# facebookresearch/metamorph

Hardware: AMD Instinct MI355X
Metric: train tokens/sec (LLaMA-3-8B + SigLIP-SO400M, seq2048, 256 img toks), whole job (higher is better)
Workload: dtype bf16

## Files before the change

metamorph_amd/csrc/gemm_bf16.hip:

```cpp
#include "gemm_common.h"
#include <type_traits>
#include <cstdlib>

namespace {

template <int TM, int TN, int FM, int FN>
MM_DEV void gemm_epilogue(f32x4 (&acc)[FM][FN], const GemmArgs& a, unsigned char* smem, int m0, int n0, int wm, int wn, int wave, int lane) {
    const int fr = lane & 15, fq = lane >> 4;
    const int M = a.M, N = a.N;
    constexpr int CPL = TN / 4;
    float* stg = (float*)smem + wave * (16 * TN);
    const uint32_t fl = a.flags;
    const int row_l = lane >> 2, col_l = (lane & 3) * CPL;
    uint16_t* Cb = (uint16_t*)a.C;
    float* Cf = (float*)a.C;
    const bool vec_ok = ((a.ldc & 7) == 0) && (!(fl & MM355_GEMM_RESIDUAL) || (a.ldr & 7) == 0);
#pragma unroll
    for (int i = 0; i < FM; ++i) {
        __builtin_amdgcn_fence(__ATOMIC_RELEASE, "wavefront");
        __builtin_amdgcn_wave_barrier();
#pragma unroll
        for (int j = 0; j < FN; ++j)
#pragma unroll
            for (int r = 0; r < 4; ++r) stg[(fq * 4 + r) * TN + j * 16 + fr] = acc[i][j][r];
// ... 8 lines not shown
                if (c >= N) continue;
                float v[8];
                const f32x4 s0 = *(const f32x4*)(stg + row_l * TN + col_l + j * 8);
                const f32x4 s1 = *(const f32x4*)(stg + row_l * TN + col_l + j * 8 + 4);
                v[0] = s0.x; v[1] = s0.y; v[2] = s0.z; v[3] = s0.w;
                v[4] = s1.x; v[5] = s1.y; v[6] = s1.z; v[7] = s1.w;
                epi_store8(a, fl, vec_ok, grow, rr, c, v);
            }
        }
    }
}

MM_DEV void gemm_epilogue_swiglu(f32x4 (&acc)[8][4], const GemmArgs& a, unsigned char* smem, int m0, int tn, int wm, int wn, int wave, int lane) {
    constexpr int TN = 64;
    const int fr = lane & 15, fq = lane >> 4;
    const int M = a.M, I = (int)a.res_mod;
    float* stg = (float*)smem + wave * (16 * TN);
    const int row_l = lane >> 2, k4 = lane & 3;
    uint16_t* gu = (uint16_t*)a.C;
    uint16_t* act = (uint16_t*)a.res;
    const int ch0 = tn * 128 + wn * 32;
#pragma unroll
    for (int i = 0; i < 8; ++i) {
        __builtin_amdgcn_fence(__ATOMIC_RELEASE, "wavefront");
        __builtin_amdgcn_wave_barrier();
#pragma unroll
        for (int j = 0; j < 4; ++j)
#pragma unroll
            for (int r = 0; r < 4; ++r) stg[(fq * 4 + r) * TN + j * 16 + fr] = acc[i][j][r];
        __builtin_amdgcn_fence(__ATOMIC_RELEASE, "wavefront");
        __builtin_amdgcn_wave_barrier();
        const int grow = m0 + wm * 128 + i * 16 + row_l;
        if (grow < M) {
            float g[8], u[8], o[8];
            const f32x4 g0 = *(const f32x4*)(stg + row_l * TN + k4 * 8), g1 = *(const f32x4*)(stg + row_l * TN + k4 * 8 + 4);
            const f32x4 u0 = *(const f32x4*)(stg + row_l * TN + 32 + k4 * 8), u1 = *(const f32x4*)(stg + row_l * TN + 32 + k4 * 8 + 4);
            g[0] = g0.x; g[1] = g0.y; g[2] = g0.z; g[3] = g0.w; g[4] = g1.x; g[5] = g1.y; g[6] = g1.z; g[7] = g1.w;
            u[0] = u0.x; u[1] = u0.y; u[2] = u0.z; u[3] = u0.w; u[4] = u1.x; u[5] = u1.y; u[6] = u1.z; u[7] = u1.w;
            const u32x4 gp = pack8(g), up = pack8(u);
            const int ch = ch0 + k4 * 8;
            *(u32x4*)(gu + (int64_t)grow * a.ldc + ch) = gp;
            *(u32x4*)(gu + (int64_t)grow * a.ldc + I + ch) = up;
            float gb[8], ub[8];
            unpack8(gp, gb);
            unpack8(up, ub);
#pragma unroll
            for (int e = 0; e < 8; ++e) o[e] = round_bf(gb[e] / (1.0f + __expf(-gb[e]))) * ub[e];
            *(u32x4*)(act + (int64_t)grow * a.ldr + ch) = pack8(o);
        }
    }
}

constexpr int SWB_TROW = 144;
constexpr int SWB_T = 3 * 32 * SWB_TROW;
constexpr int SWB_LDS = 32768 + 8 * SWB_T;
MM_DEV void gemm_epilogue_swiglu_bwd(f32x4 (&acc)[8][4], const GemmArgs& a, unsigned char* smem, int m0, int n0, int wm, int wn, int wave, int lane) {
    constexpr int TN = 64, PF = 4;
    typedef __attribute__((ext_vector_type(4))) short s16x4;
    typedef __attribute__((address_space(3))) s16x4* lds4_t;
    const int fr = lane & 15, fq = lane >> 4;
    const int M = a.M, I = a.N;
    float* stg = (float*)smem + wave * (16 * TN);
    unsigned char* tile = smem + 32768 + wave * SWB_T;
    const int row_l = lane >> 2, k4 = lane & 3;
    const uint16_t* gu = a.res;
    uint16_t* dgu = (uint16_t*)a.C;
    const int c_wave = n0 + wn * 64;
    if (c_wave >= I) return;
    const int row0 = m0 + wm * 128 + row_l;
    u32x4 gq[PF][2], uq[PF][2];
    auto fetch = [&](int i, int slot) {
        const int grow = row0 + i * 16;
#pragma unroll
        for (int j8 = 0; j8 < 2; ++j8) {
            const int64_t ro = (int64_t)min(grow, M - 1) * a.ldr + c_wave + k4 * 16 + j8 * 8;
            gq[slot][j8] = *(const u32x4*)(gu + ro);
            uq[slot][j8] = *(const u32x4*)(gu + ro + I);
        }
    };
#pragma unroll
    for (int i = 0; i < PF; ++i) fetch(i, i);
#pragma unroll
    for (int ib = 0; ib < 4; ++ib) {
#pragma unroll
        for (int half = 0; half < 2; ++half) {
            const int i = ib * 2 + half;
            __builtin_amdgcn_fence(__ATOMIC_RELEASE, "wavefront");
            __builtin_amdgcn_wave_barrier();
#pragma unroll
            for (int j = 0; j < 4; ++j)
#pragma unroll
                for (int r = 0; r < 4; ++r) stg[(fq * 4 + r) * TN + j * 16 + fr] = acc[i][j][r];
            __builtin_amdgcn_fence(__ATOMIC_RELEASE, "wavefront");
            __builtin_amdgcn_wave_barrier();
            const int grow = row0 + i * 16;
            const bool live = grow < M;
#pragma unroll
            for (int j8 = 0; j8 < 2; ++j8) {
                const int c = k4 * 16 + j8 * 8;
                float daf[8], g[8], u[8], dg[8], du[8], av[8], da[8];
                const f32x4 s0 = *(const f32x4*)(stg + row_l * TN + c), s1 = *(const f32x4*)(stg + row_l * TN + c + 4);
                daf[0] = s0.x; daf[1] = s0.y; daf[2] = s0.z; daf[3] = s0.w; daf[4] = s1.x; daf[5] = s1.y; daf[6] = s1.z; daf[7] = s1.w;
                unpack8(pack8(daf), da);
                unpack8(gq[i % PF][j8], g);
                unpack8(uq[i % PF][j8], u);
#pragma unroll
                for (int e = 0; e < 8; ++e) {
                    const float sg = 1.0f / (1.0f + __expf(-g[e]));
                    const float silu = g[e] * sg;
                    av[e] = round_bf(silu) * u[e];
                    du[e] = da[e] * round_bf(silu);
                    dg[e] = da[e] * u[e] * (sg * (1.0f + g[e] * (1.0f - sg)));
                }
                const u32x4 pg = pack8(dg), pu = pack8(du), pa = pack8(av);
                if (live) {
                    const int64_t wo = (int64_t)grow * a.ldc + c_wave + c;
                    *(u32x4*)(dgu + wo) = pg;
                    *(u32x4*)(dgu + wo + I) = pu;
                }
                unsigned char* tp = tile + (half * 16 + row_l) * SWB_TROW + c * 2;
                *(u32x4*)(tp) = pa;
                *(u32x4*)(tp + 32 * SWB_TROW) = pg;
                *(u32x4*)(tp + 64 * SWB_TROW) = pu;
            }
            if (i + PF < 8) fetch(i + PF, i % PF);
        }
        __builtin_amdgcn_fence(__ATOMIC_RELEASE, "wavefront");
        __builtin_amdgcn_wave_barrier();
        const int r_base = m0 + wm * 128 + ib * 32;
        const int s_l = fr >> 2, j_l = fr & 3;
        const unsigned char* tb = tile + (8 * (fr & 3) + (fr >> 2)) * SWB_TROW + fq * 8;
#pragma unroll
        for (int q = 0; q < 3; ++q) {
#pragma unroll
            for (int it = 0; it < 4; ++it) {
                const s16x4 lo = __builtin_amdgcn_ds_read_tr16_b64_v4i16((lds4_t)(tb + q * 32 * SWB_TROW + it * 32));
                const s16x4 hi = __builtin_amdgcn_ds_read_tr16_b64_v4i16((lds4_t)(tb + (q * 32 + 4) * SWB_TROW + it * 32));
                const int ch = c_wave + it * 16 + fq * 4 + j_l;
                const int r8 = r_base + 8 * s_l;
                if (r8 < M) {
                    typedef __attribute__((ext_vector_type(8))) short s16x8;
                    uint16_t* outp = (q == 0 ? a.aux0 : a.aux1) + (int64_t)(q == 2 ? I + ch : ch) * a.ld_aux;
                    *(s16x8*)(outp + r8) = s16x8{lo[0], lo[1], lo[2], lo[3], hi[0], hi[1], hi[2], hi[3]};
                }
            }
        }
    }
}

MM_DEV void gemm_epilogue_rope(f32x4 (&acc)[8][4], const GemmArgs& a, unsigned char* smem, int m0, int n0, int wm, int wn, int wave, int lane) {
    constexpr int TN = 64;
    const int fr = lane & 15, fq = lane >> 4;
    const int M = a.M, L = (int)a.ld_aux, n_rot = (int)a.res_mod;
    float* stg = (float*)smem + wave * (16 * TN);
    const int row_l = lane >> 2, k4 = lane & 3;
    uint16_t* out = (uint16_t*)a.C;
    const int32_t* pos_off = (const int32_t*)a.bias;
    const int d1 = (wn & 1) * 32 + k4 * 8;
    const int col1 = n0 + (wn >> 1) * 128 + d1;
    const bool rot = col1 < n_rot;
#pragma unroll
    for (int i = 0; i < 8; ++i) {
        __builtin_amdgcn_fence(__ATOMIC_RELEASE, "wavefront");
        __builtin_amdgcn_wave_barrier();
#pragma unroll
        for (int j = 0; j < 4; ++j)
#pragma unroll
            for (int r = 0; r < 4; ++r) stg[(fq * 4 + r) * TN + j * 16 + fr] = acc[i][j][r];
        __builtin_amdgcn_fence(__ATOMIC_RELEASE, "wavefront");
        __builtin_amdgcn_wave_barrier();
        const int grow = m0 + wm * 128 + i * 16 + row_l;
        if (grow < M) {
            float a1[8], a2[8], x1[8], x2[8];
            const f32x4 p0 = *(const f32x4*)(stg + row_l * TN + k4 * 8), p1 = *(const f32x4*)(stg + row_l * TN + k4 * 8 + 4);
            const f32x4 q0 = *(const f32x4*)(stg + row_l * TN + 32 + k4 * 8), q1 = *(const f32x4*)(stg + row_l * TN + 32 + k4 * 8 + 4);
            a1[0] = p0.x; a1[1] = p0.y; a1[2] = p0.z; a1[3] = p0.w; a1[4] = p1.x; a1[5] = p1.y; a1[6] = p1.z; a1[7] = p1.w;
            a2[0] = q0.x; a2[1] = q0.y; a2[2] = q0.z; a2[3] = q0.w; a2[4] = q1.x; a2[5] = q1.y; a2[6] = q1.z; a2[7] = q1.w;
            u32x4 w1 = pack8(a1), w2 = pack8(a2);
            if (rot) {
                unpack8(w1, x1);
                unpack8(w2, x2);
                const int b = grow / L;
                const int l = grow - b * L + (pos_off ? pos_off[b] : 0);
                float c[8], sn[8], y1[8], y2[8];
                unpack8(*(const u32x4*)(a.aux0 + (int64_t)l * 128 + d1), c);
                unpack8(*(const u32x4*)(a.aux1 + (int64_t)l * 128 + d1), sn);
#pragma unroll
                for (int e = 0; e < 8; ++e) {
                    y1[e] = round_bf(x1[e] * c[e]) + round_bf(-x2[e] * sn[e]);
                    y2[e] = round_bf(x2[e] * c[e]) + round_bf(x1[e] * sn[e]);
                }
                w1 = pack8(y1); w2 = pack8(y2);
            }
            *(u32x4*)(out + (int64_t)grow * a.ldc + col1) = w1;
            *(u32x4*)(out + (int64_t)grow * a.ldc + col1 + 64) = w2;
        }
    }
}

// ... 911 lines not shown

#ifdef MM355_LEGACY_VARIANTS
int launch_gemm_pp2(GemmArgs a, hipStream_t s) {
    if (!pp_eligible(a, false, false)) return launch_gemm<256, 256, 2, 4, true, 1, false>(a, s);
    static std::atomic<uint64_t> lds_ok{0};
    if (mm_ensure_dynamic_lds((const void*)gemm_pp2_kernel, PP_LDS, lds_ok) != MM355_OK) return MM355_ELAUNCH;
    const int64_t total = pp_prepare(a);
    if (total <= 0 || total > 0x7fffffff) return MM355_EINVAL;
    hipLaunchKernelGGL(gemm_pp2_kernel, dim3((unsigned)total), dim3(512), PP_LDS, s, a);
    return mm_launch_status();
}

#endif

int launch_gemm_pp(GemmArgs a, hipStream_t s) {
    if (!pp_eligible(a, false, false)) return launch_gemm<256, 256, 2, 4, true, 1, false>(a, s);
    return launch_gemm_pp_t<false, false>(a, s);
}

#ifdef MM355_LEGACY_VARIANTS
int launch_gemm_ring(GemmArgs a, hipStream_t s) {
    if (a.K < 128) return launch_gemm<256, 256, 2, 4, true, 0, false>(a, s);
    constexpr int LDS = 4 * (256 + 256) * 64;
    static std::atomic<uint64_t> lds_ok{0};
    if (mm_ensure_dynamic_lds((const void*)gemm_nt_ring_kernel, LDS, lds_ok) != MM355_OK) return MM355_ELAUNCH;
    a.ntm = (a.M + 255) / 256;
    a.ntn = (a.N + 255) / 256;
    const int64_t total = (int64_t)a.ntm * a.ntn;
    if (total <= 0 || total > 0x7fffffff) return MM355_EINVAL;
    hipLaunchKernelGGL(gemm_nt_ring_kernel, dim3((unsigned)total), dim3(512), LDS, s, a);
    return mm_launch_status();
}

#endif

template <int BM, int BN, int WM, int WN, bool GLDS, int PIPE = 0, bool TNL = false>
int launch_gemm(GemmArgs a, hipStream_t s) {
    constexpr int STAGE = (BM + BN) * 128;
    constexpr int LDS = 2 * STAGE;
    auto kern = gemm_nt_kernel<BM, BN, WM, WN, GLDS, PIPE, TNL>;
    static std::atomic<uint64_t> lds_ok{0};
    if (mm_ensure_dynamic_lds((const void*)kern, LDS, lds_ok) != MM355_OK) return MM355_ELAUNCH;
    a.ntm = (a.M + BM - 1) / BM;
    a.ntn = (a.N + BN - 1) / BN;
    const int64_t total = (int64_t)a.ntm * a.ntn;
    if (total <= 0 || total > 0x7fffffff) return MM355_EINVAL;
    hipLaunchKernelGGL(kern, dim3((unsigned)total), dim3(WM * WN * 64), LDS, s, a);
    return mm_launch_status();
}

__global__ __launch_bounds__(256) void transpose_kernel(const uint16_t* __restrict__ in, int64_t ld_in, int rows, int cols,
                                                        uint16_t* __restrict__ out, int64_t ld_out) {
    __shared__ uint16_t tile[64][64 + 2];
    const int r0 = blockIdx.y * 64, c0 = blockIdx.x * 64;
    const int tid = threadIdx.x;
#pragma unroll
    for (int i = 0; i < 2; ++i) {
        const int v = tid + i * 256, r = v >> 3, c = (v & 7) * 8;
        const int gr = r0 + r, gc = c0 + c;
        uint16_t tmp[8];
        if (gr < rows && gc + 8 <= cols) {
            *(u32x4*)tmp = *(const u32x4*)(in + (int64_t)gr * ld_in + gc);
        } else {
#pragma unroll
            for (int e = 0; e < 8; ++e) tmp[e] = (gr < rows && gc + e < cols) ? in[(int64_t)gr * ld_in + gc + e] : (uint16_t)0;
        }
#pragma unroll
        for (int e = 0; e < 8; ++e) tile[r][c + e] = tmp[e];
    }
    __syncthreads();
#pragma unroll
    for (int i = 0; i < 2; ++i) {
        const int v = tid + i * 256, c = v >> 3, r = (v & 7) * 8;
        const int gc = c0 + c, gr = r0 + r;
        if (gc >= cols) continue;
        uint16_t tmp[8];
#pragma unroll
        for (int e = 0; e < 8; ++e) tmp[e] = tile[r + e][c];
        if (gr + 8 <= rows && ((ld_out & 7) == 0)) {
            *(u32x4*)(out + (int64_t)gc * ld_out + gr) = *(const u32x4*)tmp;
        } else {
            for (int e = 0; e < 8; ++e)
                if (gr + e < rows) out[(int64_t)gc * ld_out + gr + e] = tmp[e];
        }
    }
}

__global__ __launch_bounds__(256) void colsum_kernel(const uint16_t* __restrict__ x, int64_t ld, int M, int N, float* __restrict__ out) {
    __shared__ float part[4][64];
    const int cq = threadIdx.x & 63, rp = threadIdx.x >> 6;
    const int c = blockIdx.x * 64 + cq;
    float s = 0.f;
    if (c < N)
        for (int r = rp; r < M; r += 4) s += bf2f(x[(int64_t)r * ld + c]);
    part[rp][cq] = s;
    __syncthreads();
    if (rp == 0 && c < N) out[c] += (part[0][cq] + part[1][cq]) + (part[2][cq] + part[3][cq]);
}

__global__ __launch_bounds__(1024) void colsum8_kernel(const uint16_t* __restrict__ x, int64_t ld, int M, int N, float* __restrict__ out) {
    __shared__ float part[128][65];
    const int cg = threadIdx.x & 7, rp = threadIdx.x >> 3;
    const int c0 = blockIdx.x * 64 + cg * 8;
    float s[8] = {0.f, 0.f, 0.f, 0.f, 0.f, 0.f, 0.f, 0.f};
    if (c0 < N)
        for (int r = rp; r < M; r += 128) {
            float f[8];
// ... 379 lines not shown
}
}

extern "C" int mm355_gemm_pair_bf16(const mm355_bf16* A0, int64_t lda0, const mm355_bf16* B0, int64_t ldb0, void* C0, int64_t ldc0,
                                    int64_t M0, int64_t N0, int64_t K0, uint32_t flags0,
                                    const mm355_bf16* A1, int64_t lda1, const mm355_bf16* B1, int64_t ldb1, void* C1, int64_t ldc1,
                                    int64_t M1, int64_t N1, int64_t K1, uint32_t flags1, void* stream) {
    (void)hipGetLastError();
    GemmArgs a0, a1;
    int rc = pair_problem(a0, A0, lda0, B0, ldb0, C0, ldc0, M0, N0, K0, flags0);
    if (rc != MM355_OK) return rc;
    rc = pair_problem(a1, A1, lda1, B1, ldb1, C1, ldc1, M1, N1, K1, flags1);
    if (rc != MM355_OK) return rc;
    return launch_gemm_pp_pair(a0, a1, (hipStream_t)stream);
}

extern "C" int mm355_gemm_tn_bf16(const mm355_bf16* At, int64_t lda, const mm355_bf16* Bt, int64_t ldb, void* C, int64_t ldc, int64_t M,
                                  int64_t N, int64_t K, uint32_t flags, void* stream) {
    (void)hipGetLastError();
    if (!At || !Bt || !C || M < 8 || N < 8 || K <= 0) return MM355_EINVAL;
    if ((M & 7) || (N & 7) || (lda & 7) || (ldb & 7) || !mm_aligned16(At) || !mm_aligned16(Bt) || !mm_aligned16(C)) return MM355_EINVAL;
    if (K % 64) return MM355_EUNSUPPORTED;
    if (flags & ~(MM355_GEMM_ACCUMULATE | MM355_GEMM_OUT_F32)) return MM355_EINVAL;
    if (M > 0x7fffffff || N > 0x7fffffff || K > 0x7fffffff) return MM355_EINVAL;
    GemmArgs a = {};
    a.A = At; a.B = Bt; a.C = C; a.bias = nullptr; a.res = nullptr;
    a.lda = lda; a.ldb = ldb; a.ldc = ldc; a.ldr = 0; a.res_mod = 0;
    a.M = (int)M; a.N = (int)N; a.K = (int)K; a.flags = flags; a.ntm = a.ntn = 0;
    if (pp_eligible(a, true, true)) return launch_gemm_pp_t<true, true>(a, (hipStream_t)stream);
    return launch_gemm<256, 256, 2, 4, true, 1, true>(a, (hipStream_t)stream);
}

extern "C" int mm355_gemm_nn_bf16(const mm355_bf16* A, int64_t lda, const mm355_bf16* Bt, int64_t ldb, void* C, int64_t ldc, int64_t M,
                                  int64_t N, int64_t K, const mm355_bf16* residual, int64_t ldr, uint32_t flags, void* stream) {
    (void)hipGetLastError();
    if (!A || !Bt || !C || M <= 0 || N < 8 || K <= 0) return MM355_EINVAL;
    if ((N & 7) || (lda & 7) || (ldb & 7) || (ldc & 7) || !mm_aligned16(A) || !mm_aligned16(Bt) || !mm_aligned16(C)) return MM355_EINVAL;
    if (flags & ~(MM355_GEMM_ACCUMULATE | MM355_GEMM_OUT_F32 | MM355_GEMM_RESIDUAL)) return MM355_EINVAL;
    if ((flags & MM355_GEMM_RESIDUAL) && (!residual || !mm_aligned16(residual) || (ldr & 7))) return MM355_EINVAL;
    if (M > 0x7fffffff || N > 0x7fffffff || K > 0x7fffffff) return MM355_EINVAL;
    GemmArgs a = {};
    a.A = A; a.B = Bt; a.C = C; a.bias = nullptr; a.res = residual;
    a.lda = lda; a.ldb = ldb; a.ldc = ldc; a.ldr = ldr; a.res_mod = 0;
    a.M = (int)M; a.N = (int)N; a.K = (int)K; a.flags = flags; a.ntm = a.ntn = 0;
    if (!pp_eligible(a, false, true)) return MM355_EUNSUPPORTED;
    return launch_gemm_pp_t<false, true>(a, (hipStream_t)stream);
}

extern "C" int mm355_transpose_bf16(const mm355_bf16* in, int64_t ld_in, int64_t rows, int64_t cols, mm355_bf16* out,
                                    int64_t ld_out, void* stream) {
    (void)hipGetLastError();
    if (!in || !out || rows <= 0 || cols <= 0 || (ld_in & 7) || !mm_aligned16(in) || !mm_aligned16(out)) return MM355_EINVAL;
    if (ld_out < rows || rows > 0x7fffffff || cols > 0x7fffffff) return MM355_EINVAL;
    dim3 grid((unsigned)((cols + 63) / 64), (unsigned)((rows + 63) / 64));
    hipLaunchKernelGGL(transpose_kernel, grid, dim3(256), 0, (hipStream_t)stream, in, ld_in, (int)rows, (int)cols, out, ld_out);
    return mm_launch_status();
}

extern "C" int mm355_gemm_swiglu_bf16(const mm355_bf16* X, int64_t ldx, const mm355_bf16* Wgu, int64_t ldw, mm355_bf16* gu, int64_t ld_gu,
                                      mm355_bf16* act, int64_t ld_act, int64_t M, int64_t I, int64_t K, void* stream) {
    (void)hipGetLastError();
    if (!X || !Wgu || !gu || !act || M <= 0 || I <= 0 || K <= 0) return MM355_EINVAL;
    if ((ldx & 7) || (ldw & 7) || (ld_gu & 7) || (ld_act & 7) || !mm_aligned16(X) || !mm_aligned16(Wgu) || !mm_aligned16(gu) || !mm_aligned16(act))
        return MM355_EINVAL;
    if (M > 0x7fffffff || I > 0x3fffffff || K > 0x7fffffff) return MM355_EINVAL;
    if ((I & 127) || K < 128 || (K & 127) || (2 * I * ldw + K) * 2 >= 0x7fffffffLL || (256 * ldx + K) * 2 >= 0x7fffffffLL) return MM355_EUNSUPPORTED;
    GemmArgs a = {};
    a.A = X; a.B = Wgu; a.C = gu; a.bias = nullptr; a.res = act;
    a.lda = ldx; a.ldb = ldw; a.ldc = ld_gu; a.ldr = ld_act; a.res_mod = I;
    a.M = (int)M; a.N = (int)(2 * I); a.K = (int)K; a.flags = 0; a.ntm = a.ntn = 0;
    static std::atomic<uint64_t> lds_ok{0};
    if (mm_ensure_dynamic_lds((const void*)gemm_pp_swiglu_kernel, PP_LDS, lds_ok) != MM355_OK) return MM355_ELAUNCH;
    const int64_t total = pp_prepare(a);
    if (total <= 0 || total > 0x7fffffff) return MM355_EINVAL;
    hipLaunchKernelGGL(gemm_pp_swiglu_kernel, dim3((unsigned)total), dim3(512), PP_LDS, (hipStream_t)stream, a);
    return mm_launch_status();
}

extern "C" int mm355_gemm_rope_bf16(const mm355_bf16* X, int64_t ldx, const mm355_bf16* Wqkv, int64_t ldw, mm355_bf16* qkv, int64_t ld_qkv,
                                    const mm355_bf16* cos_t, const mm355_bf16* sin_t, const int32_t* pos_offset,
                                    int64_t M, int64_t N, int64_t K, int64_t L, int64_t n_rot, void* stream) {
    (void)hipGetLastError();
    if (!X || !Wqkv || !qkv || !cos_t || !sin_t || M <= 0 || N <= 0 || K <= 0 || L <= 0 || n_rot < 0 || n_rot > N) return MM355_EINVAL;
    if ((ldx & 7) || (ldw & 7) || (ld_qkv & 7) || !mm_aligned16(X) || !mm_aligned16(Wqkv) || !mm_aligned16(qkv) || !mm_aligned16(cos_t) || !mm_aligned16(sin_t))
        return MM355_EINVAL;
    if (M > 0x7fffffff || N > 0x7fffffff || K > 0x7fffffff || L > 0x7fffffff) return MM355_EINVAL;
    if ((N & 255) || (n_rot & 127) || K < 128 || (K & 127) || (256 * ldx + K) * 2 >= 0x7fffffffLL || (256 * ldw + K) * 2 >= 0x7fffffffLL) return MM355_EUNSUPPORTED;
    GemmArgs a = {};
    a.A = X; a.B = Wqkv; a.C = qkv; a.bias = (const uint16_t*)pos_offset; a.res = nullptr;
    a.lda = ldx; a.ldb = ldw; a.ldc = ld_qkv; a.ldr = 0; a.res_mod = n_rot;
    a.M = (int)M; a.N = (int)N; a.K = (int)K; a.flags = 0; a.ntm = a.ntn = 0;
    a.aux0 = (uint16_t*)cos_t; a.aux1 = (uint16_t*)sin_t; a.ld_aux = L;
    static std::atomic<uint64_t> lds_ok{0};
    if (mm_ensure_dynamic_lds((const void*)gemm_pp_rope_kernel, PP_LDS, lds_ok) != MM355_OK) return MM355_ELAUNCH;
    const int64_t total = pp_prepare(a);
    if (total <= 0 || total > 0x7fffffff) return MM355_EINVAL;
    hipLaunchKernelGGL(gemm_pp_rope_kernel, dim3((unsigned)total), dim3(512), PP_LDS, (hipStream_t)stream, a);
    return mm_launch_status();
}

extern "C" int mm355_gemm_swiglu_bwd_bf16(const mm355_bf16* dY, int64_t ldy, const mm355_bf16* WdT, int64_t ldw, const mm355_bf16* gu, int64_t ld_gu,
                                          mm355_bf16* dgu, int64_t ld_dgu, mm355_bf16* actT, mm355_bf16* dguT, int64_t ldT,
                                          int64_t M, int64_t I, int64_t K, void* stream) {
    (void)hipGetLastError();
    if (!dY || !WdT || !gu || !dgu || !actT || !dguT || M <= 0 || I <= 0 || K <= 0) return MM355_EINVAL;
    if ((ldy & 7) || (ldw & 7) || (ld_gu & 7) || (ld_dgu & 7) || (ldT & 7) || ldT < M || !mm_aligned16(dY) || !mm_aligned16(WdT) || !mm_aligned16(gu)
        || !mm_aligned16(dgu) || !mm_aligned16(actT) || !mm_aligned16(dguT))
        return MM355_EINVAL;
// ... 26 lines not shown
```

metamorph_amd/csrc/mm355_common.h:

```cpp
#pragma once

#include <hip/hip_runtime.h>
#include <atomic>
#include <stdint.h>

#include "../../include/mm355.h"

typedef __attribute__((ext_vector_type(8))) short bf16x8;
typedef __attribute__((ext_vector_type(4))) short bf16x4;
typedef __attribute__((ext_vector_type(4))) float f32x4;
typedef __attribute__((ext_vector_type(16))) float f32x16;
typedef __attribute__((ext_vector_type(4))) uint32_t u32x4;
typedef __attribute__((ext_vector_type(2))) uint32_t u32x2;

#define MM_DEV __device__ __forceinline__

MM_DEV float bf2f(uint16_t h) { return __uint_as_float(((uint32_t)h) << 16); }
MM_DEV uint16_t f2bf(float f) {
    __bf16 b = (__bf16)f;
    return __builtin_bit_cast(uint16_t, b);
}
typedef float mm_f32x2 __attribute__((ext_vector_type(2)));
typedef __bf16 mm_bf16x2 __attribute__((ext_vector_type(2)));
MM_DEV uint32_t pack2bf(float lo, float hi) {
    return __builtin_bit_cast(uint32_t, __builtin_convertvector(mm_f32x2{lo, hi}, mm_bf16x2));
}
MM_DEV float bflo(uint32_t w) { return __uint_as_float(w << 16); }
MM_DEV float bfhi(uint32_t w) { return __uint_as_float(w & 0xffff0000u); }
MM_DEV float round_bf(float f) { return bf2f(f2bf(f)); }

MM_DEV void unpack8(const u32x4& v, float* f) {
    f[0] = bflo(v.x); f[1] = bfhi(v.x); f[2] = bflo(v.y); f[3] = bfhi(v.y);
    f[4] = bflo(v.z); f[5] = bfhi(v.z); f[6] = bflo(v.w); f[7] = bfhi(v.w);
}
MM_DEV u32x4 pack8(const float* f) {
    u32x4 v;
    v.x = pack2bf(f[0], f[1]); v.y = pack2bf(f[2], f[3]); v.z = pack2bf(f[4], f[5]); v.w = pack2bf(f[6], f[7]);
    return v;
}

MM_DEV float wave_sum(float v) {
#pragma unroll
    for (int o = 32; o > 0; o >>= 1) v += __shfl_xor(v, o, 64);
    return v;
}
MM_DEV float wave_max(float v) {
#pragma unroll
    for (int o = 32; o > 0; o >>= 1) v = fmaxf(v, __shfl_xor(v, o, 64));
    return v;
}

template <int NT>
MM_DEV float block_sum(float v, float* red) {
    v = wave_sum(v);
    const int w = threadIdx.x >> 6, l = threadIdx.x & 63;
    __syncthreads();
    if (l == 0) red[w] = v;
    __syncthreads();
    float t = 0.f;
#pragma unroll
    for (int i = 0; i < NT / 64; ++i) t += red[i];
    return t;
}
template <int NT>
MM_DEV float block_max(float v, float* red) {
    v = wave_max(v);
    const int w = threadIdx.x >> 6, l = threadIdx.x & 63;
    __syncthreads();
    if (l == 0) red[w] = v;
    __syncthreads();
    float t = red[0];
#pragma unroll
    for (int i = 1; i < NT / 64; ++i) t = fmaxf(t, red[i]);
    return t;
}

MM_DEV float gelu_erf_f(float x) { return 0.5f * x * (1.0f + erff(x * 0.70710678118654752440f)); }
MM_DEV float gelu_tanh_f(float x) {
    const float c = 0.79788456080286535588f;
    return 0.5f * x * (1.0f + tanhf(c * (x + 0.044715f * x * x * x)));
}
MM_DEV float gelu_erf_grad(float x) {
// ... 28 lines not shown
```

metamorph_amd/csrc/rowwise.hip:

```cpp
#include "mm355_common.h"
#include "rowsum.h"
#include <type_traits>

namespace {

constexpr int NT = 256;

template <int VPT>
__global__ __launch_bounds__(NT) void rmsnorm_fwd_kernel(const uint16_t* __restrict__ x, const uint16_t* __restrict__ w,
                                                         uint16_t* __restrict__ y, float* __restrict__ rstd_out, int h, float eps) {
    __shared__ float red[NT / 64];
    const int64_t row = blockIdx.x;
    const int nv = h >> 3;
    const uint16_t* xr = x + row * h;
    float xv[VPT][8];
    float ss = 0.f;
#pragma unroll
    for (int i = 0; i < VPT; ++i) {
        const int v = threadIdx.x + i * NT;
        if (v < nv) {
            unpack8(*(const u32x4*)(xr + v * 8), xv[i]);
#pragma unroll
            for (int e = 0; e < 8; ++e) ss += xv[i][e] * xv[i][e];
        }
    }
    ss = block_sum<NT>(ss, red);
    const float rstd = rsqrtf(ss / (float)h + eps);
    if (rstd_out && threadIdx.x == 0) rstd_out[row] = rstd;
#pragma unroll
    for (int i = 0; i < VPT; ++i) {
        const int v = threadIdx.x + i * NT;
        if (v < nv) {
            float wv[8], o[8];
            unpack8(*(const u32x4*)(w + v * 8), wv);
#pragma unroll
            for (int e = 0; e < 8; ++e) o[e] = wv[e] * round_bf(xv[i][e] * rstd);
            *(u32x4*)(y + row * h + v * 8) = pack8(o);
        }
    }
}

__global__ __launch_bounds__(256) void rmsnorm_apply_t_kernel(const uint16_t* __restrict__ x, const uint16_t* __restrict__ w,
                                                              const float* __restrict__ rstd, int M, int h,
                                                              uint16_t* __restrict__ out, int64_t ld_out) {
    __shared__ uint16_t tile[64][64 + 2];
    const int r0 = blockIdx.y * 64, c0 = blockIdx.x * 64;
    const int tid = threadIdx.x;
#pragma unroll
    for (int i = 0; i < 2; ++i) {
        const int v = tid + i * 256, r = v >> 3, c = (v & 7) * 8;
        const int gr = r0 + r, gc = c0 + c;
        uint16_t tmp[8];
        if (gr < M && gc + 8 <= h) {
            float xv[8], wv[8], o[8];
            unpack8(*(const u32x4*)(x + (int64_t)gr * h + gc), xv);
            unpack8(*(const u32x4*)(w + gc), wv);
            const float rs = rstd[gr];
#pragma unroll
            for (int e = 0; e < 8; ++e) o[e] = wv[e] * round_bf(xv[e] * rs);
            *(u32x4*)tmp = pack8(o);
        } else {
#pragma unroll
            for (int e = 0; e < 8; ++e) tmp[e] = 0;
        }
#pragma unroll
        for (int e = 0; e < 8; ++e) tile[r][c + e] = tmp[e];
    }
    __syncthreads();
#pragma unroll
    for (int i = 0; i < 2; ++i) {
        const int v = tid + i * 256, c = v >> 3, r = (v & 7) * 8;
        const int gc = c0 + c, gr = r0 + r;
        if (gc >= h) continue;
        uint16_t tmp[8];
#pragma unroll
        for (int e = 0; e < 8; ++e) tmp[e] = tile[r + e][c];
        if (gr + 8 <= M && ((ld_out & 7) == 0)) {
            *(u32x4*)(out + (int64_t)gc * ld_out + gr) = *(const u32x4*)tmp;
        } else {
            for (int e = 0; e < 8; ++e)
                if (gr + e < M) out[(int64_t)gc * ld_out + gr + e] = tmp[e];
        }
    }
}

template <int VPT>
__global__ __launch_bounds__(NT) void rmsnorm_bwd_kernel(const uint16_t* __restrict__ dy, const uint16_t* __restrict__ x,
                                                         const uint16_t* __restrict__ w, const uint16_t* __restrict__ dres,
                                                         uint16_t* __restrict__ dx, float* __restrict__ dw,
                                                         float* __restrict__ ws, int M, int h, float eps, int rows_per_block) {
    __shared__ float red[NT / 64];
    const int nv = h >> 3;
    float wv[VPT][8], dwacc[VPT][8];
#pragma unroll
    for (int i = 0; i < VPT; ++i) {
        const int v = threadIdx.x + i * NT;
#pragma unroll
        for (int e = 0; e < 8; ++e) { dwacc[i][e] = 0.f; wv[i][e] = 0.f; }
        if (v < nv) unpack8(*(const u32x4*)(w + v * 8), wv[i]);
// ... 411 lines not shown
        const float nrm = fmaxf(round_bf(sqrtf(ss)), 1e-12f);
        inv = 1.0f / nrm;
        dot *= inv * inv;
    }
    const float w00 = (1.0f - lx) * (1.0f - ly), w01 = lx * (1.0f - ly), w10 = (1.0f - lx) * ly, w11 = lx * ly;
    for (int v = lane; v < nv; v += 64) {
        float r[8], gy[8];
        unpack8(*(const u32x4*)(g + v * 8), gy);
        if (normalize) interp(v, r);
#pragma unroll
        for (int e = 0; e < 8; ++e) {
            const float dr = normalize ? (gy[e] - r[e] * dot) * inv : gy[e];
            if (si == so) atomicAdd(din + o00 + v * 8 + e, dr);
            else {
                atomicAdd(din + o00 + v * 8 + e, dr * w00);
                atomicAdd(din + o01 + v * 8 + e, dr * w01);
                atomicAdd(din + o10 + v * 8 + e, dr * w10);
                atomicAdd(din + o11 + v * 8 + e, dr * w11);
            }
        }
    }
}

template <typename F>
int dispatch_vpt(int h, F&& f) {
    const int nv = h >> 3;
    if (nv <= NT) return f(std::integral_constant<int, 1>{});
    if (nv <= 2 * NT) return f(std::integral_constant<int, 2>{});
    if (nv <= 4 * NT) return f(std::integral_constant<int, 4>{});
    if (nv <= 8 * NT) return f(std::integral_constant<int, 8>{});
    return MM355_EUNSUPPORTED;
}

}

extern "C" int mm355_rmsnorm_fwd_rstd(const mm355_bf16* x, const mm355_bf16* w, mm355_bf16* y, float* rstd_out, int64_t M, int64_t h, float eps,
                                      void* stream) {
    (void)hipGetLastError();
    if (!x || !w || !y || M <= 0 || h <= 0 || (h & 7) || M > 0x7fffffff) return MM355_EINVAL;
    return dispatch_vpt((int)h, [&](auto vpt) {
        hipLaunchKernelGGL((rmsnorm_fwd_kernel<decltype(vpt)::value>), dim3((unsigned)M), dim3(NT), 0, (hipStream_t)stream, x, w, y, rstd_out,
                           (int)h, eps);
        return mm_launch_status();
    });
}
extern "C" int mm355_rmsnorm_fwd(const mm355_bf16* x, const mm355_bf16* w, mm355_bf16* y, int64_t M, int64_t h, float eps, void* stream) {
    return mm355_rmsnorm_fwd_rstd(x, w, y, nullptr, M, h, eps, stream);
}
extern "C" int mm355_rmsnorm_apply_t(const mm355_bf16* x, const mm355_bf16* w, const float* rstd, int64_t M, int64_t h, mm355_bf16* out_t,
                                     int64_t ld_out, void* stream) {
    (void)hipGetLastError();
    if (!x || !w || !rstd || !out_t || M <= 0 || h <= 0 || (h & 7) || M > 0x7fffffff || ld_out < M) return MM355_EINVAL;
    if (!mm_aligned16(x) || !mm_aligned16(w) || !mm_aligned16(out_t)) return MM355_EINVAL;
    dim3 grid((unsigned)((h + 63) / 64), (unsigned)((M + 63) / 64));
    hipLaunchKernelGGL(rmsnorm_apply_t_kernel, grid, dim3(256), 0, (hipStream_t)stream, x, w, rstd, (int)M, (int)h, out_t, ld_out);
    return mm_launch_status();
}

constexpr int DWR_COLS = 32;
__global__ __launch_bounds__(256) void rmsnorm_dw_reduce_kernel(const float* __restrict__ ws, float* __restrict__ dw, int G, int h, int ld) {
    __shared__ f32x4 part[32][8];
    const int cq = threadIdx.x & 7, rl = threadIdx.x >> 3;
    const int c = blockIdx.x * DWR_COLS + cq * 4;
    f32x4 acc0 = {0.f, 0.f, 0.f, 0.f}, acc1 = {0.f, 0.f, 0.f, 0.f};
    if (c < h) {
        const float* p = ws + c;
        int g = rl;
        for (; g + 32 < G; g += 64) {
            acc0 += *(const f32x4*)(p + (int64_t)g * ld);
            acc1 += *(const f32x4*)(p + (int64_t)(g + 32) * ld);
        }
        if (g < G) acc0 += *(const f32x4*)(p + (int64_t)g * ld);
    }
    part[rl][cq] = acc0 + acc1;
    __syncthreads();
    if (rl == 0 && c < h) {
        f32x4 s = part[0][cq];
#pragma unroll
        for (int r = 1; r < 32; ++r) s += part[r][cq];
#pragma unroll
        for (int e = 0; e < 4; ++e) dw[c + e] += s[e];
    }
}

__global__ __launch_bounds__(256) void rmsnorm_dw_reduce_bf16_kernel(const float* __restrict__ ws, uint16_t* __restrict__ grad, int G, int h, int ld,
                                                                     int accumulate) {
    __shared__ f32x4 part[32][8];
    const int cq = threadIdx.x & 7, rl = threadIdx.x >> 3;
    const int c = blockIdx.x * DWR_COLS + cq * 4;
    f32x4 acc0 = {0.f, 0.f, 0.f, 0.f}, acc1 = {0.f, 0.f, 0.f, 0.f};
    if (c < h) {
        const float* p = ws + c;
        int g = rl;
        for (; g + 32 < G; g += 64) {
            acc0 += *(const f32x4*)(p + (int64_t)g * ld);
            acc1 += *(const f32x4*)(p + (int64_t)(g + 32) * ld);
        }
        if (g < G) acc0 += *(const f32x4*)(p + (int64_t)g * ld);
    }
    part[rl][cq] = acc0 + acc1;
    __syncthreads();
    if (rl == 0 && c < h) {
        f32x4 s = part[0][cq];
#pragma unroll
        for (int r = 1; r < 32; ++r) s += part[r][cq];
#pragma unroll
        for (int e = 0; e < 4; ++e) grad[c + e] = f2bf(s[e] + (accumulate ? bf2f(grad[c + e]) : 0.f));
    }
// ... 134 lines not shown
```

Before: 26210.

## Restructure SwiGLU backward epilogue staging and swizzle transpose tile order

The SwiGLU backward GEMM epilogue now stages the accumulator as bf16 through a transposed LDS tile, reads it back with ds_read_tr, and emits transposed aux outputs in 64-row halves. The separate fp32 staging buffer is gone, which shrinks LDS use, and the global loads for gate and up are rearranged into row-major 8-row pieces. The transpose kernels switch to a 1D grid whose tiles are grouped into bands of four column tiles to improve write locality when there are many column tiles. The change also adds debug macros (MM355_SWB_EPI) that skip the loads or the stores, but they are off by default.

New measurement: 26420 (median of 6 runs). About the same (+0.8%).

```diff
diff --git a/metamorph_amd/csrc/gemm_bf16.hip b/metamorph_amd/csrc/gemm_bf16.hip
--- a/metamorph_amd/csrc/gemm_bf16.hip
+++ b/metamorph_amd/csrc/gemm_bf16.hip
@@ -84,99 +84,105 @@
 }
 
 constexpr int SWB_TROW = 144;
-constexpr int SWB_T = 3 * 32 * SWB_TROW;
-constexpr int SWB_LDS = 32768 + 8 * SWB_T;
+constexpr int SWB_T = 2 * 64 * SWB_TROW;
+constexpr int SWB_LDS = 8 * SWB_T;
 MM_DEV void gemm_epilogue_swiglu_bwd(f32x4 (&acc)[8][4], const GemmArgs& a, unsigned char* smem, int m0, int n0, int wm, int wn, int wave, int lane) {
-    constexpr int TN = 64, PF = 4;
+    constexpr int PF = 4;
     typedef __attribute__((ext_vector_type(4))) short s16x4;
+    typedef __attribute__((ext_vector_type(8))) short s16x8;
     typedef __attribute__((address_space(3))) s16x4* lds4_t;
     const int fr = lane & 15, fq = lane >> 4;
+    const int s_l = fr >> 2, j_l = fr & 3;
     const int M = a.M, I = a.N;
-    float* stg = (float*)smem + wave * (16 * TN);
-    unsigned char* tile = smem + 32768 + wave * SWB_T;
-    const int row_l = lane >> 2, k4 = lane & 3;
+    unsigned char* tD = smem + wave * SWB_T;
+    unsigned char* tQ = tD + 64 * SWB_TROW;
     const uint16_t* gu = a.res;
     uint16_t* dgu = (uint16_t*)a.C;
     const int c_wave = n0 + wn * 64;
     if (c_wave >= I) return;
-    const int row0 = m0 + wm * 128 + row_l;
-    u32x4 gq[PF][2], uq[PF][2];
-    auto fetch = [&](int i, int slot) {
-        const int grow = row0 + i * 16;
-#pragma unroll
-        for (int j8 = 0; j8 < 2; ++j8) {
-            const int64_t ro = (int64_t)min(grow, M - 1) * a.ldr + c_wave + k4 * 16 + j8 * 8;
-            gq[slot][j8] = *(const u32x4*)(gu + ro);
-            uq[slot][j8] = *(const u32x4*)(gu + ro + I);
-        }
-    };
-#pragma unroll
-    for (int i = 0; i < PF; ++i) fetch(i, i);
-#pragma unroll
-    for (int ib = 0; ib < 4; ++ib) {
-#pragma unroll
-        for (int half = 0; half < 2; ++half) {
-            const int i = ib * 2 + half;
-            __builtin_amdgcn_fence(__ATOMIC_RELEASE, "wavefront");
-            __builtin_amdgcn_wave_barrier();
-#pragma unroll
-            for (int j = 0; j < 4; ++j)
-#pragma unroll
-                for (int r = 0; r < 4; ++r) stg[(fq * 4 + r) * TN + j * 16 + fr] = acc[i][j][r];
-            __builtin_amdgcn_fence(__ATOMIC_RELEASE, "wavefront");
-            __builtin_amdgcn_wave_barrier();
-            const int grow = row0 + i * 16;
-            const bool live = grow < M;
-#pragma unroll
-            for (int j8 = 0; j8 < 2; ++j8) {
-                const int c = k4 * 16 + j8 * 8;
-                float daf[8], g[8], u[8], dg[8], du[8], av[8], da[8];
-                const f32x4 s0 = *(const f32x4*)(stg + row_l * TN + c), s1 = *(const f32x4*)(stg + row_l * TN + c + 4);
-                daf[0] = s0.x; daf[1] = s0.y; daf[2] = s0.z; daf[3] = s0.w; daf[4] = s1.x; daf[5] = s1.y; daf[6] = s1.z; daf[7] = s1.w;
-                unpack8(pack8(daf), da);
-                unpack8(gq[i % PF][j8], g);
-                unpack8(uq[i % PF][j8], u);
-#pragma unroll
-                for (int e = 0; e < 8; ++e) {
-                    const float sg = 1.0f / (1.0f + __expf(-g[e]));
-                    const float silu = g[e] * sg;
-                    av[e] = round_bf(silu) * u[e];
-                    du[e] = da[e] * round_bf(silu);
-                    dg[e] = da[e] * u[e] * (sg * (1.0f + g[e] * (1.0f - sg)));
-                }
-                const u32x4 pg = pack8(dg), pu = pack8(du), pa = pack8(av);
-                if (live) {
-                    const int64_t wo = (int64_t)grow * a.ldc + c_wave + c;
-                    *(u32x4*)(dgu + wo) = pg;
-                    *(u32x4*)(dgu + wo + I) = pu;
-                }
-                unsigned char* tp = tile + (half * 16 + row_l) * SWB_TROW + c * 2;
-                *(u32x4*)(tp) = pa;
-                *(u32x4*)(tp + 32 * SWB_TROW) = pg;
-                *(u32x4*)(tp + 64 * SWB_TROW) = pu;
-            }
-            if (i + PF < 8) fetch(i + PF, i % PF);
-        }
+    const int rw0 = m0 + wm * 128;
+    const int kc = s_l + 4 * (fq & 1), prow = 4 * (fq >> 1) + j_l;
+    const unsigned char* dsup = tD + (8 * ((fr & 3) + 4 * (fq & 1)) + (fr >> 2)) * SWB_TROW + 8 * (fq >> 1);
+    const unsigned char* qsup = tQ + (32 * (fq & 1) + 8 * (fr & 3) + (fr >> 2)) * SWB_TROW + 8 * (fq >> 1);
+    u32x4 gq[PF], uq[PF];
+    auto fetch = [&](int p, int slot) {
+        const int64_t ro = (int64_t)min(rw0 + p * 8 + prow, M - 1) * a.ldr + c_wave + kc * 8;
+#if defined(MM355_SWB_EPI) && MM355_SWB_EPI == 2
+        const uint32_t cv = 0x3f003f00u ^ (uint32_t)(ro & 0x00ff00ff);
+        gq[slot] = u32x4{cv, cv, cv, cv};
+        uq[slot] = u32x4{cv ^ 0x10001u, cv, cv, cv};
+#else
+        gq[slot] = *(const u32x4*)(gu + ro);
+        uq[slot] = *(const u32x4*)(gu + ro + I);
+#endif
+    };
+    auto fence = [] {
         __builtin_amdgcn_fence(__ATOMIC_RELEASE, "wavefront");
         __builtin_amdgcn_wave_barrier();
-        const int r_base = m0 + wm * 128 + ib * 32;
-        const int s_l = fr >> 2, j_l = fr & 3;
-        const unsigned char* tb = tile + (8 * (fr & 3) + (fr >> 2)) * SWB_TROW + fq * 8;
-#pragma unroll
-        for (int q = 0; q < 3; ++q) {
-#pragma unroll
-            for (int it = 0; it < 4; ++it) {
-                const s16x4 lo = __builtin_amdgcn_ds_read_tr16_b64_v4i16((lds4_t)(tb + q * 32 * SWB_TROW + it * 32));
-                const s16x4 hi = __builtin_amdgcn_ds_read_tr16_b64_v4i16((lds4_t)(tb + (q * 32 + 4) * SWB_TROW + it * 32));
-                const int ch = c_wave + it * 16 + fq * 4 + j_l;
-                const int r8 = r_base + 8 * s_l;
-                if (r8 < M) {
-                    typedef __attribute__((ext_vector_type(8))) short s16x8;
-                    uint16_t* outp = (q == 0 ? a.aux0 : a.aux1) + (int64_t)(q == 2 ? I + ch : ch) * a.ld_aux;
-                    *(s16x8*)(outp + r8) = s16x8{lo[0], lo[1], lo[2], lo[3], hi[0], hi[1], hi[2], hi[3]};
-                }
+    };
+    auto flush = [&](uint16_t* out, int r0) {
+        fence();
+#if !(defined(MM355_SWB_EPI) && MM355_SWB_EPI == 1)
+        const int r8 = r0 + 32 * (fq & 1) + 8 * s_l;
+#pragma unroll
+        for (int cg = 0; cg < 8; ++cg) {
+            const s16x4 lo = __builtin_amdgcn_ds_read_tr16_b64_v4i16((lds4_t)(qsup + cg * 16));
+            const s16x4 hi = __builtin_amdgcn_ds_read_tr16_b64_v4i16((lds4_t)(qsup + 4 * SWB_TROW + cg * 16));
+            if (r8 < M)
+                *(s16x8*)(out + (int64_t)(cg * 8 + 4 * (fq >> 1) + j_l) * a.ld_aux + r8) = s16x8{lo[0], lo[1], lo[2], lo[3], hi[0], hi[1], hi[2], hi[3]};
+        }
+#endif
+        fence();
+    };
+#pragma unroll
+    for (int p = 0; p < PF; ++p) fetch(p, p);
+#pragma unroll
+    for (int hb = 0; hb < 2; ++hb) {
+        fence();
+#pragma unroll
+        for (int il = 0; il < 4; ++il)
+#pragma unroll
+            for (int j = 0; j < 4; ++j) {
+                const f32x4 v = acc[4 * hb + il][j];
+                *(u32x2*)(tD + (16 * j + fr) * SWB_TROW + (16 * il + 4 * fq) * 2) = u32x2{pack2bf(v.x, v.y), pack2bf(v.z, v.w)};
             }
-        }
+        fence();
+        u32x4 PG[8], PU[8];
+#pragma unroll
+        for (int p8 = 0; p8 < 8; ++p8) {
+            const int p = hb * 8 + p8, row = rw0 + p * 8 + prow;
+            const s16x4 dlo = __builtin_amdgcn_ds_read_tr16_b64_v4i16((lds4_t)(dsup + p8 * 16));
+            const s16x4 dhi = __builtin_amdgcn_ds_read_tr16_b64_v4i16((lds4_t)(dsup + 4 * SWB_TROW + p8 * 16));
+            float g[8], u[8], dg[8], du[8], av[8], da[8];
+            unpack8(__builtin_bit_cast(u32x4, s16x8{dlo[0], dlo[1], dlo[2], dlo[3], dhi[0], dhi[1], dhi[2], dhi[3]}), da);
+            unpack8(gq[p % PF], g);
+            unpack8(uq[p % PF], u);
+            if (p + PF < 16) fetch(p + PF, p % PF);
+#pragma unroll
+            for (int e = 0; e < 8; ++e) {
+                const float sg = 1.0f / (1.0f + __expf(-g[e]));
+                const float silu = g[e] * sg;
+                av[e] = round_bf(silu) * u[e];
+                du[e] = da[e] * round_bf(silu);
+                dg[e] = da[e] * u[e] * (sg * (1.0f + g[e] * (1.0f - sg)));
+            }
+            PG[p8] = pack8(dg);
+            PU[p8] = pack8(du);
+            if (row < M) {
+                const int64_t wo = (int64_t)row * a.ldc + c_wave + kc * 8;
+                *(u32x4*)(dgu + wo) = PG[p8];
+                *(u32x4*)(dgu + wo + I) = PU[p8];
+            }
+            *(u32x4*)(tQ + (p8 * 8 + prow) * SWB_TROW + kc * 16) = pack8(av);
+        }
+        const int r0 = rw0 + hb * 64;
+        flush(a.aux0 + (int64_t)c_wave * a.ld_aux, r0);
+#pragma unroll
+        for (int p8 = 0; p8 < 8; ++p8) *(u32x4*)(tQ + (p8 * 8 + prow) * SWB_TROW + kc * 16) = PG[p8];
+        flush(a.aux1 + (int64_t)c_wave * a.ld_aux, r0);
+#pragma unroll
+        for (int p8 = 0; p8 < 8; ++p8) *(u32x4*)(tQ + (p8 * 8 + prow) * SWB_TROW + kc * 16) = PU[p8];
+        flush(a.aux1 + (int64_t)(I + c_wave) * a.ld_aux, r0);
     }
 }
 
@@ -1194,7 +1200,9 @@
 __global__ __launch_bounds__(256) void transpose_kernel(const uint16_t* __restrict__ in, int64_t ld_in, int rows, int cols,
                                                         uint16_t* __restrict__ out, int64_t ld_out) {
     __shared__ uint16_t tile[64][64 + 2];
-    const int r0 = blockIdx.y * 64, c0 = blockIdx.x * 64;
+    int ct, rt;
+    transpose_tile_of(blockIdx.x, (cols + 63) / 64, (rows + 63) / 64, ct, rt);
+    const int r0 = rt * 64, c0 = ct * 64;
     const int tid = threadIdx.x;
 #pragma unroll
     for (int i = 0; i < 2; ++i) {
@@ -1680,8 +1688,9 @@
     (void)hipGetLastError();
     if (!in || !out || rows <= 0 || cols <= 0 || (ld_in & 7) || !mm_aligned16(in) || !mm_aligned16(out)) return MM355_EINVAL;
     if (ld_out < rows || rows > 0x7fffffff || cols > 0x7fffffff) return MM355_EINVAL;
-    dim3 grid((unsigned)((cols + 63) / 64), (unsigned)((rows + 63) / 64));
-    hipLaunchKernelGGL(transpose_kernel, grid, dim3(256), 0, (hipStream_t)stream, in, ld_in, (int)rows, (int)cols, out, ld_out);
+    const int64_t tiles = ((cols + 63) / 64) * ((rows + 63) / 64);
+    if (tiles > 0x7fffffff) return MM355_EINVAL;
+    hipLaunchKernelGGL(transpose_kernel, dim3((unsigned)tiles), dim3(256), 0, (hipStream_t)stream, in, ld_in, (int)rows, (int)cols, out, ld_out);
     return mm_launch_status();
 }
 
diff --git a/metamorph_amd/csrc/mm355_common.h b/metamorph_amd/csrc/mm355_common.h
--- a/metamorph_amd/csrc/mm355_common.h
+++ b/metamorph_amd/csrc/mm355_common.h
@@ -28,6 +28,15 @@
 MM_DEV float bflo(uint32_t w) { return __uint_as_float(w << 16); }
 MM_DEV float bfhi(uint32_t w) { return __uint_as_float(w & 0xffff0000u); }
 MM_DEV float round_bf(float f) { return bf2f(f2bf(f)); }
+
+MM_DEV void transpose_tile_of(int b, int nct, int nrt, int& ct, int& rt) {
+    if (nct <= 128) { ct = b % nct; rt = b / nct; return; }
+    constexpr int G = 4;
+    const int band = b / (G * nrt), in = b - band * G * nrt;
+    const int gw = min(G, nct - band * G);
+    ct = band * G + in % gw;
+    rt = in / gw;
+}
 
 MM_DEV void unpack8(const u32x4& v, float* f) {
     f[0] = bflo(v.x); f[1] = bfhi(v.x); f[2] = bflo(v.y); f[3] = bfhi(v.y);
diff --git a/metamorph_amd/csrc/rowwise.hip b/metamorph_amd/csrc/rowwise.hip
--- a/metamorph_amd/csrc/rowwise.hip
+++ b/metamorph_amd/csrc/rowwise.hip
@@ -44,7 +44,9 @@
                                                               const float* __restrict__ rstd, int M, int h,
                                                               uint16_t* __restrict__ out, int64_t ld_out) {
     __shared__ uint16_t tile[64][64 + 2];
-    const int r0 = blockIdx.y * 64, c0 = blockIdx.x * 64;
+    int ct, rt;
+    transpose_tile_of(blockIdx.x, (h + 63) / 64, (M + 63) / 64, ct, rt);
+    const int r0 = rt * 64, c0 = ct * 64;
     const int tid = threadIdx.x;
 #pragma unroll
     for (int i = 0; i < 2; ++i) {
@@ -562,8 +564,9 @@
     (void)hipGetLastError();
     if (!x || !w || !rstd || !out_t || M <= 0 || h <= 0 || (h & 7) || M > 0x7fffffff || ld_out < M) return MM355_EINVAL;
     if (!mm_aligned16(x) || !mm_aligned16(w) || !mm_aligned16(out_t)) return MM355_EINVAL;
-    dim3 grid((unsigned)((h + 63) / 64), (unsigned)((M + 63) / 64));
-    hipLaunchKernelGGL(rmsnorm_apply_t_kernel, grid, dim3(256), 0, (hipStream_t)stream, x, w, rstd, (int)M, (int)h, out_t, ld_out);
+    const int64_t tiles = ((h + 63) / 64) * ((M + 63) / 64);
+    if (tiles > 0x7fffffff) return MM355_EINVAL;
+    hipLaunchKernelGGL(rmsnorm_apply_t_kernel, dim3((unsigned)tiles), dim3(256), 0, (hipStream_t)stream, x, w, rstd, (int)M, (int)h, out_t, ld_out);
     return mm_launch_status();
 }
 
```
